# uci-rendering/psdr-cuda

Measured on AMD Instinct MI355X. Metric: Mpath-samples/s renderC+renderD, cbox 512x512 spp=64; grad rel-L2 vs ref, higher is better.
Workload: dtype f32

## Files before the change

psdr-cuda_amd/csrc/psdr_device.h:

```cpp
#pragma once
#include "psdr_math.h"
#include "../../include/psdr_hip.h"

namespace psdr {

struct __attribute__((aligned(16))) BvhNode {
    float lo0[3], hi0[3];
    float lo1[3], hi1[3];
    int32_t c0, c1;
    int32_t pad[2];
};
static_assert(sizeof(BvhNode) == 64, "BvhNode must be 64 bytes");

struct __attribute__((aligned(16))) Bvh4Node {
    float org[3];
    uint32_t exps;
    uint32_t qlo[3], qhi[3];
    int32_t child[4];
    uint32_t pad[2];
};
static_assert(sizeof(Bvh4Node) == 64, "Bvh4Node must be 64 bytes");
constexpr int32_t kNoChild = 0x7ffffffe;

constexpr int kBvhStack = 40;
// ... 980 lines not shown
    const float iw = 1.f / v[3];
    const Vec3f d = normalize(Vec3f{v[0] * iw, v[1] * iw, v[2] * iw});
    const float *c = sc.d.cam + PSDR_CAM_TO_WORLD;
    constexpr auto tm = &psdr_tangents::d_cam_to_world;
    auto tw = [&](int r, int col) { if constexpr (is_ad<R>()) return ldf<R>(c, tv, tm, r * 4 + col); else return R(uniform_word(c, r * 4 + col)); };
    RayT<R> ray;
    const R w = tw(3, 3);
    ray.o = Vec3<R>(tw(0, 3) / w, tw(1, 3) / w, tw(2, 3) / w);
    ray.d = Vec3<R>(tw(0, 0) * d.x + tw(0, 1) * d.y + tw(0, 2) * d.z, tw(1, 0) * d.x + tw(1, 1) * d.y + tw(1, 2) * d.z,
                    tw(2, 0) * d.x + tw(2, 1) * d.y + tw(2, 2) * d.z);
    return ray;
}
PSDR_HD bool sample_direct(const SceneView &sc, const Vec3f &p, int &pixel, float &qx, float &qy, float &sensor_val) {
    const float *m = sc.d.cam + PSDR_CAM_WORLD_TO_SAMPLE;
    float v[4];
#pragma unroll
    for (int r = 0; r < 4; ++r) v[r] = m[r * 4] * p.x + m[r * 4 + 1] * p.y + m[r * 4 + 2] * p.z + m[r * 4 + 3];
    qx = v[0] / v[3]; qy = v[1] / v[3];
    const int W = sc.d.width, H = sc.d.height;
    const int ix = (int) floorf(qx * (float) W), iy = (int) floorf(qy * (float) H);
    const bool ok = ix >= 0 && ix < W && iy >= 0 && iy < H;
    pixel = ok ? iy * W + ix : -1;
    const float *c = sc.d.cam;
    Vec3f dir{p.x - c[PSDR_CAM_POS], p.y - c[PSDR_CAM_POS + 1], p.z - c[PSDR_CAM_POS + 2]};
    const float d2 = dot(dir, dir);
    dir = dir / sqrtf(fmaxf(d2, 0.f));
    const float ict = 1.f / (c[PSDR_CAM_DIR] * dir.x + c[PSDR_CAM_DIR + 1] * dir.y + c[PSDR_CAM_DIR + 2] * dir.z);
    sensor_val = (1.f / d2) * (ict * ict * ict) * c[PSDR_CAM_INV_AREA];
    return ok;
}

#ifndef PSDR_EMITTER_PRETEST
#define PSDR_EMITTER_PRETEST 1
#endif
#ifndef PSDR_SKIP_UNLIT
#define PSDR_SKIP_UNLIT 1
#endif
#ifndef PSDR_OCC_ROWS
#define PSDR_OCC_ROWS 1
#endif
template <class R> PSDR_HD R mis_weight(const R &p1, const R &p2) { const R a = sqr(p1), b = sqr(p2); return a / (a + b); }

struct LiParams {
    int integrator, bsdf_samples, light_samples, max_depth, hide_emitters, field;
};

template <class R> PSDR_HD void copy_its(Its<R> &d, const Its<R> &a) {
    d.valid = a.valid; d.tri = a.tri; d.mesh = a.mesh; d.hu = a.hu; d.hv = a.hv;
    d.wi.x = a.wi.x; d.wi.y = a.wi.y; d.wi.z = a.wi.z; d.p.x = a.p.x; d.p.y = a.p.y; d.p.z = a.p.z; d.n.x = a.n.x; d.n.y = a.n.y; d.n.z = a.n.z;
    d.t = a.t; d.J = a.J; d.uvx = a.uvx; d.uvy = a.uvy;
    d.sh.s.x = a.sh.s.x; d.sh.s.y = a.sh.s.y; d.sh.s.z = a.sh.s.z; d.sh.t.x = a.sh.t.x; d.sh.t.y = a.sh.t.y; d.sh.t.z = a.sh.t.z;
    d.sh.n.x = a.sh.n.x; d.sh.n.y = a.sh.n.y; d.sh.n.z = a.sh.n.z;
}
template <class NI, class G> PSDR_HD NI its_cast(const Its<G> &a) {
    if constexpr (std::is_same<NI, Its<G>>::value) { if constexpr (is_ad<G>()) { NI r; copy_its(r, a); return r; } else return a; }
    else {
        Its<float> r;
        r.valid = a.valid; r.tri = a.tri; r.mesh = a.mesh; r.hu = a.hu; r.hv = a.hv;
        r.wi = val(a.wi); r.p = val(a.p); r.n = val(a.n); r.t = val(a.t); r.J = val(a.J); r.uvx = val(a.uvx); r.uvy = val(a.uvy);
        r.sh.s = val(a.sh.s); r.sh.t = val(a.sh.t); r.sh.n = val(a.sh.n);
        return r;
    }
}
template <class G, class M, class TVT, class NI = Its<G>>
PSDR_HD Vec3<M> direct_step(const SceneView &sc, const TVT &tv, TraversalStack &st, Rng &rng, const Its<G> &its, bool active, int nB,
                            int nL, uint32_t &nrays, NI *next_its, Vec3<M> *next_f, bool *next_valid, int *light_tri = nullptr, bool emitter_only = false) {
    constexpr bool ad = is_ad<M>();
    constexpr HitForm form = is_ad<G>() ? kPathSpace : kDetached;
    Vec3<M> result = zero3<M>();
    int bsdf_id = active ? Tab<TVT::flags>::mesh_bsdf(sc, its.mesh) : 0;
    if (bsdf_id < 0) { active = false; bsdf_id = 0; }
    const Bsdf<G, M> bsdf(sc, tv, bsdf_id);
    auto bsdf_sample = [&](const float (&s)[3], int i) {
        Vec3f wo_s; M pdf_s;
        bool a1 = bsdf.sample(sc, tv, its, s, active, wo_s, pdf_s);
        const Vec3f dir1 = val(its.sh.s) * wo_s.x + val(its.sh.t) * wo_s.y + val(its.sh.n) * wo_s.z;
        if constexpr (!TVT::has_env && TVT::forest && PSDR_EMITTER_PRETEST && !is_ad<G>()) {
            if (emitter_only && sc.emit_rows != 0u && a1) a1 = closest_hit<false, 2, true>(sc, st, val(its.p), dir1, INFINITY, -1, -1, 0, sc.emit_rows).tri >= 0;
        }
        const RayT<G> ray1{its.p, lift<G>(dir1)};
        const Its<G> its1 = intersect<G>(sc, tv, st, ray1, a1, form, nrays, -1, -1, kPreBsdfRay);
        const bool a_hit = a1 && its1.valid;
        a1 = a_hit && emitter_of(sc, tv, its1) >= 0;
        Vec3<M> bsdf_val = zero3<M>(); M pdf0(0.f);
        if (a_hit) {
            if constexpr (ad) {
                const Vec3<G> wo = (its1.p - its.p) / its1.t;
                bsdf_val = bsdf.eval(sc, tv, its, its.sh.to_local(wo), true);
                const G Gv = abs_(dot(its1.n, -wo)) / sqr(its1.t);
                pdf0 = pdf_s * val(Gv);
                bsdf_val = bsdf_val * (to_m<M>(Gv * its1.J) / pdf0);
            } else {
                bsdf_val = bsdf.eval(sc, tv, its, lift<G>(wo_s), true);
                const G Gv = abs_(dot(its1.n, -ray1.d)) / sqr(its1.t);
                pdf0 = pdf_s * Gv;
                bsdf_val = bsdf_val / pdf_s;
            }
        }
        if (a1) {
            M w(1.f / (float) nB);
            if (nL > 0) w = w * mis_weight(pdf0, M(emitter_position_pdf(sc, tv, val(its.p), its1)));
            result = result + Le<M>(sc, tv, its1, true) * bsdf_val * w;
        }
        if (next_its && i == 0) { *next_its = its_cast<NI>(its1); *next_f = bsdf_val; *next_valid = a_hit; }
    };
    auto light_sample = [&](float s0, float s1, int i) {
        const PosSample<G> ps = sample_emitter_position<G>(sc, tv, val(its.p), s0, s1, is_ad<G>());
        Vec3<G> wo = ps.p - its.p;
// ... 106 lines not shown
    const float ix = rho.x.v != 0.f ? 1.f / rho.x.v : 0.f, iy = rho.y.v != 0.f ? 1.f / rho.y.v : 0.f, iz = rho.z.v != 0.f ? 1.f / rho.z.v : 0.f;
#pragma unroll
    for (int k = 0; k < K; ++k) { g[k][0] = rho.x.d[k] * ix; g[k][1] = rho.y.d[k] * iy; g[k][2] = rho.z.d[k] * iz; }
}
template <int K, class TVT>
PSDR_HD Vec3<Dual<K>> li_path_logd(const SceneView &sc, const TVT &tv, TraversalStack &st, const LiParams &lp, Rng &rng, const RayT<float> &ray, uint32_t &nrays) {
    const TangentView<0, TVT::flags> tv0{};
    Its<float> its = intersect<float>(sc, tv0, st, ray, true, kDetached, nrays, -1, -1, kPrePrimaryRay);
    bool active = its.valid;
    Vec3f result = lp.hide_emitters ? Vec3f(0.f) : Le<float>(sc, tv0, its, active);
    float rd[K][3], s[K][3];
#pragma unroll
    for (int k = 0; k < K; ++k) { rd[k][0] = rd[k][1] = rd[k][2] = 0.f; s[k][0] = s[k][1] = s[k][2] = 0.f; }
    Vec3f beta(1.f);
    for (int depth = 0; depth < lp.max_depth; ++depth) {
        Its<float> nits; Vec3f nf; bool nvalid = false;
        if (active) {
            float g[K][3];
            albedo_logd<K>(sc, tv, its, g);
#pragma unroll
            for (int k = 0; k < K; ++k) { s[k][0] += g[k][0]; s[k][1] += g[k][1]; s[k][2] += g[k][2]; }
        }
        const Vec3f c = direct_step<float, float>(sc, tv0, st, rng, its, active, 1, 1, nrays, &nits, &nf, &nvalid, nullptr, depth + 1 >= lp.max_depth);
        if (active) {
            const Vec3f bc = beta * c;
            result = result + bc;
#pragma unroll
            for (int k = 0; k < K; ++k) {
                rd[k][0] = fmaf(bc.x, s[k][0], rd[k][0]); rd[k][1] = fmaf(bc.y, s[k][1], rd[k][1]); rd[k][2] = fmaf(bc.z, s[k][2], rd[k][2]);
            }
            active = nvalid;
            if (active) {
                beta = beta * nf;
                its = nits;
                if (!(beta.x != 0.f || beta.y != 0.f || beta.z != 0.f)) active = false;
            }
        }
    }
    Vec3<Dual<K>> out;
    out.x.v = result.x; out.y.v = result.y; out.z.v = result.z;
#pragma unroll
    for (int k = 0; k < K; ++k) { out.x.d[k] = rd[k][0]; out.y.d[k] = rd[k][1]; out.z.d[k] = rd[k][2]; }
    return out;
}
template <int K, class TVT>
PSDR_HD Vec3<Dual<K>> camera_sample_logd(const SceneView &sc, const TVT &tv, TraversalStack &st, const LiParams &lp, const RngJump &jump, int pixel, uint64_t slot, uint32_t &nrays) {
    Rng rng; rng.init(slot, jump);
    const float j0 = rng.next(), j1 = rng.next();
    const int W = sc.d.width;
    const float sx = ((float) (pixel % W) + j0) / (float) W, sy = ((float) (pixel / W) + j1) / (float) sc.d.height;
    const TangentView<0, TVT::flags> tv0{};
    const RayT<float> ray = primary_ray<float>(sc, tv0, sx, sy);
    return zero_nonfinite(li_path_logd<K>(sc, tv, st, lp, rng, ray, nrays));
}


template <class M, class TVT>
PSDR_HD Vec3<M> wavefront_camera_vertex(const SceneView &sc, const TVT &tv, TraversalStack &st, const LiParams &lp, const RngJump &jump,
                                        int pixel, uint64_t slot, uint32_t &nrays, Its<float> &next, Vec3<M> &beta, Vec3f &origin, bool &alive, Rng *rng_after = nullptr) {
    Rng rng; rng.init(slot, jump);
    const float j0 = rng.next(), j1 = rng.next();
    const int W = sc.d.width;
    const float sx = ((float) (pixel % W) + j0) / (float) W, sy = ((float) (pixel / W) + j1) / (float) sc.d.height;
    const RayT<float> ray = primary_ray<float>(sc, tv, sx, sy);
    const Its<float> its = intersect<float>(sc, tv, st, ray, true, kDetached, nrays);
    alive = false;
    if (!its.valid) return zero3<M>();
    Vec3<M> result = lp.hide_emitters ? zero3<M>() : Le<M>(sc, tv, its, true);
    bool nvalid = false;
    result = result + direct_step<float, M>(sc, tv, st, rng, its, true, 1, 1, nrays, &next, &beta, &nvalid, nullptr, lp.max_depth <= 1);
    if (rng_after) *rng_after = rng;
    origin = its.p;
    if (nvalid) { const Vec3f b = val(beta); alive = b.x != 0.f || b.y != 0.f || b.z != 0.f; }
    return result;
}
template <class M, class TVT>
PSDR_HD Vec3<M> wavefront_primary_vertex(const SceneView &sc, const TVT &tv, TraversalStack &st, const LiParams &lp, const RngJump &jump,
                                         int pixel, uint64_t slot, uint32_t &nrays, Its<float> &next, Vec3f &dir, bool &alive, Rng *rng_after = nullptr, float *sxy = nullptr) {
    Rng rng; rng.init(slot, jump);
    const float j0 = rng.next(), j1 = rng.next();
    if (rng_after) *rng_after = rng;
    const int W = sc.d.width;
    const float sx = ((float) (pixel % W) + j0) / (float) W, sy = ((float) (pixel / W) + j1) / (float) sc.d.height;
    if (sxy) { sxy[0] = sx; sxy[1] = sy; }
    const RayT<float> ray = primary_ray<float>(sc, tv, sx, sy);
    const Its<float> its = intersect<float>(sc, tv, st, ray, true, kDetached, nrays);
    alive = its.valid;
    if (!its.valid) return zero3<M>();
    next = its;
    { const Vec3f d = its.p - ray.o; dir = d / norm(d); }
    return lp.hide_emitters ? zero3<M>() : Le<M>(sc, tv, its, true);
}
template <class G> PSDR_HD Its<float> detach_its(const Its<G> &a) {
    Its<float> r;
    r.valid = a.valid; r.tri = a.tri; r.mesh = a.mesh; r.hu = a.hu; r.hv = a.hv;
    r.wi = val(a.wi); r.p = val(a.p); r.n = val(a.n); r.t = val(a.t); r.J = val(a.J); r.uvx = val(a.uvx); r.uvy = val(a.uvy);
    r.sh.s = val(a.sh.s); r.sh.t = val(a.sh.t); r.sh.n = val(a.sh.n);
    return r;
}
template <class M, class TVT>
PSDR_HD Vec3<M> wavefront_bounce_vertex(const SceneView &sc, const TVT &tv, TraversalStack &st, const RngJump &jump_k, uint64_t slot,
                                        const Its<float> &its, uint32_t &nrays, Its<float> &next, Vec3<M> &f, bool &alive, int *light_tri = nullptr,
                                        Rng *rng_after = nullptr, bool last = false) {
    Rng rng; rng.init(slot, jump_k);
    bool nvalid = false;
    if (light_tri) *light_tri = -1;
// ... 257 lines not shown
```

psdr-cuda_amd/csrc/psdr_hip.hip:

```cpp
#define PSDR_WIDE_TREE 2
#include "psdr_host.h"
#include "psdr_bvh_build.h"

#include <cstdlib>
#include <cstring>
#include <rocprim/rocprim.hpp>

namespace {
__global__ __launch_bounds__(kBlock) void k_trace(LaunchCtx cx, int m, const float *__restrict__ ox, const float *__restrict__ oy,
                                                  const float *__restrict__ oz, const float *__restrict__ dx,
                                                  const float *__restrict__ dy, const float *__restrict__ dz,
                                                  const float *__restrict__ tmax, int32_t *__restrict__ out_shape,
                                                  int32_t *__restrict__ out_tri, float *__restrict__ out_u, float *__restrict__ out_v) {
    TraversalStack st; setup_lds(cx, st);
    const SceneView &sc = cx.sc;
    for (int i = blockIdx.x * kBlock + threadIdx.x; i < m; i += gridDim.x * kBlock) {
        const Hit h = closest_hit<false, -1>(sc, st, Vec3f{ox[i], oy[i], oz[i]}, Vec3f{dx[i], dy[i], dz[i]}, tmax[i]);
        out_tri[i] = h.tri;
        out_shape[i] = h.tri >= 0 ? (sc.d.tri_mesh[h.tri] & ~PSDR_TRI_FACE_NORMALS) : -1;
        out_u[i] = h.u; out_v[i] = h.v;
    }
}


// ... 784 lines not shown
    HIP_TRY(hipMemsetAsync(pb.count, 0, cnt_bytes, s));
    return 0;
}

const VariantOps *variant_of(const psdr_scene_s *h) {
    int fl = (h->desc.env_emitter >= 0 ? kSceneEnv : 0) | (h->has_rough ? kSceneRough : 0) | (h->n_blas > 0 ? kSceneForest : 0);
    if (tiny_tables_ok(h)) fl |= kSceneTiny;
    switch (fl) {
        case 0: return variant_ops_0();
        case 1: return variant_ops_1();
        case 2: return variant_ops_2();
        case 3: return variant_ops_3();
        case 4: return variant_ops_4();
        case 8: return variant_ops_8();
        case 10: return variant_ops_10();
        default: return variant_ops_6();
    }
}
}
using namespace psdr_host;

extern "C" {

const char *psdr_last_error(void) { return g_err.c_str(); }
const char *psdr_version(void) { return "psdr-hip 0.1 gfx950"; }
int psdr_abi_struct_sizes(int32_t out[4]) {
    out[0] = (int32_t) sizeof(psdr_scene_desc); out[1] = (int32_t) sizeof(psdr_render_opts);
    out[2] = (int32_t) sizeof(psdr_tangents); out[3] = (int32_t) sizeof(psdr_grads);
    return 0;
}

int psdr_scene_create(psdr_scene_t *out) {
    if (!out) return fail("psdr_scene_create: null output");
    psdr_scene_s *h = new psdr_scene_s();
    hipError_t e = hipMalloc(&h->d_counters, sizeof(unsigned long long) * kRayCounters * kRayCounterStride);
    if (e != hipSuccess) { delete h; return fail(std::string("hipMalloc: ") + hipGetErrorString(e)); }
    int dev = 0; hipDeviceProp_t prop;
    if (hipGetDevice(&dev) == hipSuccess && hipGetDeviceProperties(&prop, dev) == hipSuccess) {
        h->num_cus = prop.multiProcessorCount;
        h->lds_limit = (int) std::min<size_t>(prop.sharedMemPerBlock, 160 * 1024);
    }
    *out = h;
    return 0;
}

int psdr_scene_set_option(psdr_scene_t h, const char *name, double value) {
    if (!h || !name) return fail("psdr_scene_set_option: null argument");
    const std::string n(name);
    const int iv = (int) value;
    if (n == "bvh_refit") h->refit_enabled = iv != 0;
    else if (n == "forest_min_inline") { h->forest_min_inline = iv; h->have_bvh = false; }
    else if (n == "scratch_plain") g_scratch_plain = iv;
    else if (n == "own_pixels") h->opt.own_pixels = iv;
    else if (n == "emitter_pretest") h->opt.emitter_pretest = iv;
    else if (n == "occ_rows") { h->opt.occ_rows = iv; h->have_bvh = false; }
    else if (n == "aa_prims") { h->aa_enabled = iv != 0; h->have_bvh = false; }
    else if (n == "tiny_scene") h->tiny_enabled = iv != 0;
    else if (n == "two_level") h->two_level_enabled = iv != 0;
    else if (n == "wf_binned") h->wf_binned = iv != 0;
    else if (n == "wf_traced") h->traced_enabled = iv != 0;
    else if (n == "bvh_build") h->bvh_device_mode = iv;
    else if (n == "sort_edges") h->sort_edges = iv != 0;
    else if (n == "blocks_per_cu") h->opt.blocks_per_cu = iv;
    else if (n == "camera_blocks") h->opt.camera_blocks = iv;
    else if (n == "tiny_variants") h->opt.tiny_variants = iv;
    else if (n == "wide") h->opt.wide = iv;
    else if (n == "lds_budget") h->opt.lds_budget = iv;
    else if (n == "sink_rep") h->opt.sink_rep = std::max(1, std::min(16, iv));
    else if (n == "sink_private") h->opt.sink_private = iv;
    else if (n == "rev_split") h->opt.rev_split = iv;
    else if (n == "tangent_live") h->opt.tangent_live = iv;
    else if (n == "wf_geo") h->opt.wf_geo = iv;
    else if (n == "logd") h->opt.logd = iv;
    else if (n == "keep_records") h->opt.keep_records = iv;
    else if (n == "rev_sorted") h->opt.rev_sorted = iv;
    else if (n == "sedge_split") h->opt.sedge_split = iv;
    else if (n == "probe") h->opt.probe = iv;
    else if (n == "trace_wg2") h->opt.trace_wg2 = iv;
    else if (n == "chunk_log2") h->opt.chunk_log2 = std::max(0, std::min(30, iv));
    else if (n == "bvh_maxleaf") h->opt.bvh_maxleaf = std::max(1, std::min(8, iv));
    else if (n == "bvh_tcost") h->opt.bvh_tcost = (float) value;
    else return fail("psdr_scene_set_option: unknown option '" + n + "'");
    h->kept.valid = false;
    if (n == "tiny_scene" || n == "two_level" || n == "bvh_build" || n == "wide" || n == "bvh_maxleaf" || n == "bvh_tcost" || n == "tiny_variants") h->have_bvh = false;
    return 0;
}

int psdr_scene_destroy(psdr_scene_t h) {
    if (!h) return 0;
    if (h->d_nodes) (void) hipFree(h->d_nodes);
    if (h->d_btris) (void) hipFree(h->d_btris);
    if (h->d_counters) (void) hipFree(h->d_counters);
    if (h->d_refit_area) (void) hipFree(h->d_refit_area);
    if (h->d_sort) (void) hipFree(h->d_sort);
    if (h->d_ws) (void) hipFree(h->d_ws);
    if (h->d_live) (void) hipFree(h->d_live);
    if (h->d_logd_bad) (void) hipFree(h->d_logd_bad);
    if (h->d_hot_map) (void) hipFree(h->d_hot_map);
    if (h->d_hot_tris) (void) hipFree(h->d_hot_tris);
    if (h->d_occ) (void) hipFree(h->d_occ);
    if (h->d_top) (void) hipFree(h->d_top);
    if (h->d_inline_ids) (void) hipFree(h->d_inline_ids);
    if (h->d_lbvh) (void) hipFree(h->d_lbvh);
    if (h->d_nodes4) (void) hipFree(h->d_nodes4);
    if (h->d_topo4) (void) hipFree(h->d_topo4);
    if (h->d_rev) (void) hipFree(h->d_rev);
// ... 371 lines not shown
```

psdr-cuda_amd/csrc/psdr_host.h:

```cpp
#pragma once
#include "psdr_device.h"
#include "psdr_reverse.h"

#include <algorithm>
#include <type_traits>
#include <cmath>
#include <cstdio>
#include <cstdlib>
#include <cstring>
#include <string>
#include <vector>

using namespace psdr;

struct LaunchCtx {
    SceneView sc;
    LiParams lp;
    RngJump jump;
    int32_t off_stack;
    int32_t off_pathrec;
    int32_t off_sink;
};

static_assert(offsetof(LaunchCtx, sc) == 0, "closest_hit reads SceneView::tiny through the kernel-argument segment pointer: LaunchCtx (SceneView first) must be the first kernel argument");
// ... 51 lines not shown
template <class TVT> __device__ __forceinline__ void setup_lds(const LaunchCtx &cx, TraversalStack &st, const TVT &tv) {
    setup_lds(cx, st);
#if defined(__HIP_DEVICE_COMPILE__)
    if constexpr (Tab<TVT::flags>::lds_small && TVT::k > 0) {
        constexpr int K = TVT::k;
        static_assert(K <= 3, "plan_lds reserves three tangent texel pools");
        if (cx.sc.lt_tex >= 0) {
            float *l = reinterpret_cast<float *>(psdr_dyn_lds + cx.sc.lt_tex);
            const int nt = cx.sc.d.num_texels;
            for (int k = 0; k < K; ++k) {
                const float *g = tv.t[k].d_texels;
                for (int i = threadIdx.x; i < nt; i += kBlock) l[(k + 1) * nt + i] = g ? g[i] : 0.f;
            }
            __syncthreads();
        }
    }
#endif
}

constexpr int kSinkCacheWords = 6144;
struct SinkLayout {
    int tex_off, tex_n;
    int rad_off, rad_n;
    int cam_off;
    int env_off, env_n;
    int hot_off, hot_rows;
    const int32_t *hot_map, *hot_tris;
    int total;
    int rep, stride;
    int priv_off, priv_rows;
    int priv_tri[2], priv_slot[2], priv_emitter;
    int priv_regs;
    int pend_off, pend_rows;
};
constexpr int kPendWords = 10;
constexpr int kPrivRowWords = 13;
constexpr int kPrivWords = 2 * kPrivRowWords + 3;

struct psdr_scene_options {
    int blocks_per_cu = 0;
    int camera_blocks = 0;
    int tiny_variants = 1;
    int wide = -1;
    int lds_budget = 0;
    int sink_rep = 4;
    int sink_private = 1;
    int rev_split = -1;
    int tangent_live = 1;
    int wf_geo = 1;
    int own_pixels = 1;
    int emitter_pretest = 1;
    int occ_rows = 1;
    int logd = 1;
    int keep_records = 1;
    int rev_sorted = 1;
    int sedge_split = -1;
    int chunk_log2 = 0;
    int probe = 1;
    int trace_wg2 = -1;
    int bvh_maxleaf = 4;
    float bvh_tcost = 2.0f;
};

struct psdr_scene_s {
    psdr_scene_options opt;
    psdr_scene_desc desc{};
    bool have_tables = false;
    bool has_rough = true;
    int num_cus = 256;
    int lds_limit = 64 * 1024;

    BvhNode *d_nodes = nullptr;
    float4 *d_btris = nullptr;
    size_t cap_nodes = 0, cap_btris = 0;
    int32_t root = 0;
    bool have_bvh = false;
    int bvh_depth = 0, num_nodes = 0, num_btris = 0;
    Bvh4Node *d_nodes4 = nullptr;
    int32_t *d_topo4 = nullptr;
    size_t cap_nodes4 = 0;
    int num_nodes4 = 0, stack_need4 = 0;
    bool wide = false;
    int32_t *d_trace_ovf = nullptr;
    size_t trace_ovf_bytes = 0;
    bool traced_enabled = true;
    int32_t root4 = 0, blas_root4[kMaxBlas] = {};
    bool refit_enabled = true;
    int tree_tris = -1, refits_since_build = 0, num_builds = 0, num_refits = 0;
    std::vector<int> level_start;
    float bvh_pad = 0.f, built_area = 0.f;
    float *d_refit_area = nullptr;

    int bvh_device_mode = -1;
    bool lbvh = false;
    int lbvh_leaves = 0;
    void *d_lbvh = nullptr;
    size_t lbvh_bytes = 0;

    bool tiny_enabled = true, aa_enabled = true;
    int n_tiny = 0, aa_cnt = 0;
    float4 tiny[kTinyRows * 4] = {};
    int32_t tiny_meta[kTinyRows * 4] = {};
    bool two_level_enabled = true, refit_ok = true, wf_binned = true;
    int n_blas = 0, n_inline = 0;
    float4 blas_lo[kMaxBlas] = {}, blas_hi[kMaxBlas] = {};
    float4 *d_top = nullptr;
// ... 92 lines not shown
```

psdr-cuda_amd/csrc/psdr_kernels.h:

```cpp
#pragma once
#include "psdr_host.h"

namespace {
using namespace psdr_host;

__device__ __forceinline__ float wave_shfl_down(float v, int off) { return __shfl_down(v, off, 64); }

template <int CTRL, int ROW_MASK> __device__ __forceinline__ float dpp_add(float v) {
    return v + __int_as_float(__builtin_amdgcn_update_dpp(0, __float_as_int(v), CTRL, ROW_MASK, 0xf, true));
}
__device__ __forceinline__ float wave_total(float v) {
    v = dpp_add<0x111, 0xf>(v); v = dpp_add<0x112, 0xf>(v); v = dpp_add<0x114, 0xf>(v); v = dpp_add<0x118, 0xf>(v);
    v = dpp_add<0x142, 0xa>(v); v = dpp_add<0x143, 0xc>(v);
    return __int_as_float(__builtin_amdgcn_readlane(__float_as_int(v), 63));
}
#ifndef PSDR_DPP_ALWAYS
#define PSDR_DPP_ALWAYS 0
#endif
template <int N, bool DPP = (N <= 6 || PSDR_DPP_ALWAYS)> __device__ __forceinline__ bool wave_segmented_sum(int key, float (&v)[N]) {
    const int lane = threadIdx.x & 63;
    if (DPP && __ballot(key != __builtin_amdgcn_readfirstlane(key)) == 0ull) {
#pragma unroll
        for (int i = 0; i < N; ++i) v[i] = wave_total(v[i]);
        return lane == 0;
// ... 147 lines not shown
    const int i = blockIdx.x * kBlock + threadIdx.x;
    bool b = false;
    if (i < n) {
        bool moved = false;
#pragma unroll
        for (int k = 0; k < K; ++k) moved = moved || tv.t[k].d_texels[i] != 0.f;
        b = moved && !(fabsf(texels[i]) > 1e-20f);
    }
    if (__ballot(b) != 0ull && (threadIdx.x & 63) == 0) atomicOr(bad, 1);
}
__global__ void k_logd_gate(unsigned long long *counters, const int *bad) { if (threadIdx.x == 0 && blockIdx.x == 0) counters[kLogdGateWord] = *bad ? 0ull : 1ull; }
template <int K, int FL, bool NOTREE>
__global__ __launch_bounds__(kBlock, ((PSDR_LOGD_WAVES_K1 > 0 && K == 1 && NOTREE) ? PSDR_LOGD_WAVES_K1 : camera_waves<float, Dual<K>, PSDR_INTEGRATOR_PATH, FL, NOTREE>())) void k_camera_logd(LaunchCtx cx, TV<Dual<K>, FL> tv, int spp, int s_begin, SlotDiv nsp,
                                                   long long n, float inv_spp, float *__restrict__ img, float *__restrict__ dimg, long long plane, unsigned long long *counters, int own) {
    constexpr int NV = 3 * (1 + K);
    if (counters[kLogdGateWord] != 1ull) return;
    TraversalStack st; setup_lds(cx, st, tv);
    uint32_t nrays = 0;
    const long long nceil = (n + kBlock - 1) / kBlock * kBlock;
    for (long long j = (long long) blockIdx.x * kBlock + threadIdx.x; j < nceil; j += (long long) gridDim.x * kBlock) {
        const bool in = j < n;
        int pixel = 0x7fffffff, s_in = 0;
        if (in) slot_to_pixel(j, nsp, pixel, s_in);
        float v[NV];
#pragma unroll
        for (int i = 0; i < NV; ++i) v[i] = 0.f;
        if (in) {
            const uint64_t slot = (uint64_t) pixel * (uint64_t) spp + (uint64_t) (s_begin + s_in);
            const Vec3<Dual<K>> r = camera_sample_logd<K>(cx.sc, tv, st, cx.lp, cx.jump, pixel, slot, nrays);
            v[0] = r.x.v * inv_spp; v[1] = r.y.v * inv_spp; v[2] = r.z.v * inv_spp;
#pragma unroll
            for (int k = 0; k < K; ++k) { v[3 + 3 * k] = r.x.d[k] * inv_spp; v[4 + 3 * k] = r.y.d[k] * inv_spp; v[5 + 3 * k] = r.z.d[k] * inv_spp; }
        }
        const bool head = wave_segmented_sum<NV>(pixel, v);
        if (head && in) {
            float *p = img + (size_t) pixel * 3;
            if (own) {
                p[0] = v[0]; p[1] = v[1]; p[2] = v[2];
#pragma unroll
                for (int k = 0; k < K; ++k) { float *q = dimg + (size_t) k * plane + (size_t) pixel * 3; q[0] = v[3 + 3 * k]; q[1] = v[4 + 3 * k]; q[2] = v[5 + 3 * k]; }
            } else {
                if (v[0] != 0.f) atomicAdd(p, v[0]);
                if (v[1] != 0.f) atomicAdd(p + 1, v[1]);
                if (v[2] != 0.f) atomicAdd(p + 2, v[2]);
#pragma unroll
                for (int k = 0; k < K; ++k) {
                    float *q = dimg + (size_t) k * plane + (size_t) pixel * 3;
                    if (v[3 + 3 * k] != 0.f) atomicAdd(q, v[3 + 3 * k]);
                    if (v[4 + 3 * k] != 0.f) atomicAdd(q + 1, v[4 + 3 * k]);
                    if (v[5 + 3 * k] != 0.f) atomicAdd(q + 2, v[5 + 3 * k]);
                }
            }
        }
    }
    count_rays(counters, nrays);
}

constexpr int kWfGroups = 16, kWfClasses = 4, kWfGrab = 8;
constexpr int kWfStageInts = (kWfSub + 1) * kWfCountStride;
struct PathStream {
    int32_t *pixel; uint32_t *slot; int32_t *tri; float *hu, *hv; float *dir; float *beta;
    float *acc;
    long long cap;
    int32_t *count;
    long long sub_cap;
    int32_t binned;
    float4 *hit;
    float *prev_t;
};
constexpr int kWfClsShift = 29;
constexpr int32_t kWfTriMask = (1 << kWfClsShift) - 1;
struct TraceQueue {
    float4 *req;
    int32_t *count;
    long long sub_cap;
};
struct WfRec {
    float *disk; long long stride;
    int spp, s_begin, nsp; long long j0;
    int stage;
    __device__ __forceinline__ long long column(int pixel, uint32_t slot) const {
        return (long long) pixel * nsp + (long long) (slot - (uint32_t) pixel * (uint32_t) spp - (uint32_t) s_begin) - j0;
    }
};

template <class M>
__device__ __forceinline__ void stream_write(const PathStream &out, long long i, int pixel, uint32_t slot, const Its<float> &next, const Vec3f &dir, const Vec3<M> &beta,
                                             const Vec3<M> &acc, int cls = 0) {
    constexpr int K = ad_traits<M>::K;
    out.pixel[i] = pixel; out.slot[i] = slot; out.tri[i] = next.tri | (cls << kWfClsShift); out.hu[i] = next.hu; out.hv[i] = next.hv;
    out.dir[i] = dir.x; out.dir[out.cap + i] = dir.y; out.dir[2 * out.cap + i] = dir.z;
    out.beta[i] = val(beta.x); out.beta[out.cap + i] = val(beta.y); out.beta[2 * out.cap + i] = val(beta.z);
    out.acc[i] = val(acc.x); out.acc[out.cap + i] = val(acc.y); out.acc[2 * out.cap + i] = val(acc.z);
#pragma unroll
    for (int k = 0; k < K; ++k) {
        out.beta[(3 + 3 * k) * out.cap + i] = tangent(beta.x, k); out.beta[(4 + 3 * k) * out.cap + i] = tangent(beta.y, k);
        out.beta[(5 + 3 * k) * out.cap + i] = tangent(beta.z, k);
        out.acc[(3 + 3 * k) * out.cap + i] = tangent(acc.x, k); out.acc[(4 + 3 * k) * out.cap + i] = tangent(acc.y, k);
        out.acc[(5 + 3 * k) * out.cap + i] = tangent(acc.z, k);
    }
}

template <class M>
__device__ __forceinline__ void stream_push(const PathStream &out, bool alive, int pixel, uint32_t slot, const Its<float> &next,
                                            const Vec3f &dir, const Vec3<M> &beta, const Vec3<M> &acc) {
    const unsigned long long mask = __ballot(alive);
// ... 1207 lines not shown
int run_camera(psdr_scene_s *h, const psdr_render_opts *o, const TV<R, FL> &tv, float *img, float *dimg, hipStream_t s) {
    const long long WH = (long long) h->desc.width * h->desc.height;
    const int nsp = o->spp_end - o->spp_begin;
    if (o->spp <= 0 || nsp <= 0) return 0;
    LaunchCtx cx;
    if (int rc = make_ctx(h, o, 0, cx)) return rc;
    const long long n = WH * nsp;
    h->slots[0] += (uint64_t) n;
    const int own = (h->opt.own_pixels != 0 && nsp <= 64 && 64 % nsp == 0) ? 1 : 0;
    if constexpr ((FL & kSceneForest) != 0) {
        if (o->integrator == PSDR_INTEGRATOR_DIRECT && probe_direct(h, o, n)) {
            const TangentView<0, FL> tv0{};
            TV<R, FL | kScenePre> tvp;
            for (int k = 0; k < (ad_traits<R>::K > 0 ? ad_traits<R>::K : 1); ++k) tvp.t[k] = tv.t[k];
            tvp.live = tv.live;
            LaunchCtx cxp = cx;
            plan_lds(h, cxp, 1 << 30);
            cxp.sc.n_lnodes = cxp.sc.n_lbtris = cxp.sc.n_ltri = 0;
            const long long chunk = std::min<long long>(n, launch_chunk(h, 25));
            for (long long c0 = 0; c0 < n; c0 += chunk) {
                const long long nc = std::min(chunk, n - c0);
                ProbeBuffers pb;
                const int probe_per_cu = big_launch_per_cu(h, nc);
                if (int rc = probe_buffers(h, nc, 3, pb, s, probe_per_cu)) return rc;
                const TraceQueue tq{pb.req, pb.count, pb.sub_cap};
                const int blocks = (launch_blocks(h, nc, probe_per_cu) + kWfSub - 1) / kWfSub * kWfSub;
                hipLaunchKernelGGL(k_direct_probe<FL>, dim3(blocks), dim3(kBlock), lds_bytes(cx, h), s, cx, tv0, o->spp, o->spp_begin, SlotDiv(nsp), c0, nc, tq, pb.hit, pb.mask,
                                   make_rng_jump(o->rng_offset[0] + 2));
                HIP_TRY(hipGetLastError());
                if (int rc = launch_wf_trace(h, pb.req, pb.count, pb.sub_cap, pb.hit, s)) return rc;
                hipLaunchKernelGGL(HIP_KERNEL_NAME(k_camera<G, R, PSDR_INTEGRATOR_DIRECT, FL | kScenePre, false>), dim3(launch_blocks(h, nc, camera_blocks_per_cu(h, nc))), dim3(kBlock), cxp.off_stack, s,
                                   cxp, tvp, o->spp, o->spp_begin, SlotDiv(nsp), nc, 1.f / (float) o->spp, img, dimg, WH * 3, h->d_counters, c0, ProbeView{pb.hit, pb.mask}, own);
                HIP_TRY(hipGetLastError());
            }
            return 0;
        }
    }
    bool gated = false;
    if constexpr (logd_instance<G, R, PSDR_INTEGRATOR_PATH, FL>()) {
        constexpr int K = ad_traits<R>::K;
        bool texels_only = o->integrator == PSDR_INTEGRATOR_PATH && h->opt.logd != 0 && h->desc.num_texels > 0 && h->desc.texels != nullptr;
        for (int k = 0; k < K && texels_only; ++k) {
            const psdr_tangents &t = tv.t[k];
            texels_only = t.d_texels != nullptr && !t.d_tri_info && !t.d_emitter_rad && !t.d_cam_to_world && !t.d_sec_edge && !t.d_prim_edge && !t.d_env_f;
        }
        if (texels_only) {
            if (int rc = scratch_reserve(&h->d_logd_bad, &h->logd_bad_bytes, sizeof(int), s, "log-derivative gate")) return rc;
            int *bad = reinterpret_cast<int *>(h->d_logd_bad);
            HIP_TRY(hipMemsetAsync(bad, 0, sizeof(int), s));
            TangentView<K, 0> tvk;
            for (int k = 0; k < K; ++k) tvk.t[k] = tv.t[k];
            hipLaunchKernelGGL(k_logd_check<K>, dim3((unsigned) ((h->desc.num_texels + kBlock - 1) / kBlock)), dim3(kBlock), 0, s, h->desc.texels, tvk, h->desc.num_texels, h->d_counters, bad);
            hipLaunchKernelGGL(k_logd_gate, dim3(1), dim3(64), 0, s, h->d_counters, bad);
            hipLaunchKernelGGL(HIP_KERNEL_NAME(k_camera_logd<K, FL, ((FL & kSceneTiny) != 0)>), dim3(launch_blocks(h, n, camera_blocks_per_cu(h, n))), dim3(kBlock), lds_bytes(cx, h), s, cx, tv,
                               o->spp, o->spp_begin, SlotDiv(nsp), n, 1.f / (float) o->spp, img, dimg, WH * 3, h->d_counters, own);
            HIP_TRY(hipGetLastError());
            gated = true;
        }
    }
#define PSDR_LAUNCH_CAMERA_T(INTEG, NOTREE)                                                                                        \
    hipLaunchKernelGGL(HIP_KERNEL_NAME(k_camera<G, R, INTEG, FL, NOTREE>), dim3(launch_blocks(h, n, camera_blocks_per_cu(h, n))), dim3(kBlock), lds_bytes(cx, h), s, cx, tv, o->spp, \
                       o->spp_begin, nsp, n, 1.f / (float) o->spp, img, dimg, WH * 3, h->d_counters, 0ll, ProbeView{nullptr, nullptr}, own)
#define PSDR_LAUNCH_CAMERA(INTEG) PSDR_LAUNCH_CAMERA_T(INTEG, ((FL & kSceneTiny) != 0))
    switch (o->integrator) {
        case PSDR_INTEGRATOR_DIRECT: PSDR_LAUNCH_CAMERA(PSDR_INTEGRATOR_DIRECT); break;
        case PSDR_INTEGRATOR_PATH: PSDR_LAUNCH_CAMERA(PSDR_INTEGRATOR_PATH); break;
        case PSDR_INTEGRATOR_FIELD: PSDR_LAUNCH_CAMERA(PSDR_INTEGRATOR_FIELD); break;
        default: return fail("Unknown integrator");
    }
#undef PSDR_LAUNCH_CAMERA
#undef PSDR_LAUNCH_CAMERA_T
    HIP_TRY(hipGetLastError());
    if (gated) HIP_TRY(hipMemsetAsync(h->d_counters + kLogdGateWord, 0, sizeof(unsigned long long), s));
    return 0;
}


constexpr int kWfMaxDepth = 256;
struct WfRecArgs { float *disk; long long stride, c0, nc; };
template <class M, int FL>
int run_camera_wavefront(psdr_scene_s *h, const psdr_render_opts *o, const TV<M, FL> &tv, float *img, float *dimg, hipStream_t s, const WfRecArgs *rec = nullptr) {
    constexpr int K = ad_traits<M>::K;
    const long long WH = (long long) h->desc.width * h->desc.height;
    const int nsp = o->spp_end - o->spp_begin;
    if (o->spp <= 0 || nsp <= 0) return 0;
    const long long n_all = WH * nsp;
    const long long n = rec ? rec->nc : n_all;
    bool traced = false;
    if constexpr ((FL & kSceneForest) != 0) traced = traced_wavefront(h);
    const bool binned = !traced && (FL & kSceneForest) != 0 && h->n_blas > 0 && h->wf_binned;
    const int depth = o->max_depth;
    const size_t words = 8 + 6 * (1 + K) + (traced ? 8 : 0);
    const long long cap = rec ? n : std::min(n, fit_chunk(binned ? launch_chunk(h, 24) : launch_chunk(h, traced ? 26 : 25), 2 * words * 4 * 5 / 4 + (traced ? 80 : 0), 64u << 20, h->ws_bytes));
    const auto wf_per_cu = [&](long long slots) { return traced ? big_launch_per_cu(h, slots) : 16; };
    const long long max_blocks = ((long long) launch_blocks(h, cap, wf_per_cu(cap)) + kWfSub - 1) / kWfSub * kWfSub;
    const long long binned_sub_cap = (((cap + kBlock - 1) / kBlock + kWfSub) / kWfGroups + 2) * kBlock;
    const long long cap_alloc = ((binned ? binned_sub_cap * kWfSub : cap + max_blocks * kBlock) + 63) / 64 * 64;
    const size_t cnt_ints = (size_t) (kWfMaxDepth + 1) * kWfStageInts + (traced ? (size_t) (kWfMaxDepth + 1) * kWfSub * kWfCountStride : 0);
    const size_t cnt_bytes = cnt_ints * sizeof(int32_t);
    const size_t req_bytes = traced ? (size_t) 2 * cap_alloc * 2 * sizeof(float4) : 0;
    const size_t need = 2 * words * 4 * (size_t) cap_alloc + cnt_bytes + req_bytes;
    if (int rc = workspace_reserve(h, need, s)) return rc;
    int32_t *cnt = reinterpret_cast<int32_t *>(h->d_ws);
    int32_t *req_cnt = cnt + (size_t) (kWfMaxDepth + 1) * kWfStageInts;
    PathStream st[2];
    for (int i = 0; i < 2; ++i) {
        float *b = reinterpret_cast<float *>(reinterpret_cast<char *>(h->d_ws) + cnt_bytes) + (size_t) i * words * cap_alloc;
        const long long c = cap_alloc;
        st[i].cap = c;
        st[i].pixel = reinterpret_cast<int32_t *>(b); st[i].slot = reinterpret_cast<uint32_t *>(b + c); st[i].tri = reinterpret_cast<int32_t *>(b + 2 * c);
        st[i].hu = b + 3 * c; st[i].hv = b + 4 * c; st[i].dir = b + 5 * c; st[i].beta = b + 8 * c; st[i].acc = b + (8 + 3 * (1 + K)) * c;
        st[i].hit = traced ? reinterpret_cast<float4 *>(b + (8 + 6 * (1 + K)) * c) : nullptr;
        st[i].prev_t = nullptr;
        st[i].binned = binned ? 1 : 0;
    }
    TraceQueue tq{};
    tq.req = traced ? reinterpret_cast<float4 *>(reinterpret_cast<char *>(h->d_ws) + cnt_bytes + 2 * words * 4 * (size_t) cap_alloc) : nullptr;
// ... 558 lines not shown
```

Measured before the change: 19970.

## Add compact path-tracing camera kernels with reduced state for tiny scenes

Adds specialized camera kernels for the primal and log-derivative path integrators on tiny scenes without a tree or environment map. Between bounces they carry only a minimal next-hit record (tri, u, v) instead of a full intersection struct, and they can park the per-path derivative sums in LDS. The kernels set launch bounds and an SGPR cap to raise occupancy. This trades extra LDS traffic and a second code path to maintain for lower register pressure, and they are on by default via compact_path=3.

```diff
diff --git a/psdr-cuda_amd/csrc/psdr_device.h b/psdr-cuda_amd/csrc/psdr_device.h
--- a/psdr-cuda_amd/csrc/psdr_device.h
+++ b/psdr-cuda_amd/csrc/psdr_device.h
@@ -1056,8 +1056,10 @@
     d.sh.s.x = a.sh.s.x; d.sh.s.y = a.sh.s.y; d.sh.s.z = a.sh.s.z; d.sh.t.x = a.sh.t.x; d.sh.t.y = a.sh.t.y; d.sh.t.z = a.sh.t.z;
     d.sh.n.x = a.sh.n.x; d.sh.n.y = a.sh.n.y; d.sh.n.z = a.sh.n.z;
 }
+struct NextHit { int tri; float u, v; };
 template <class NI, class G> PSDR_HD NI its_cast(const Its<G> &a) {
-    if constexpr (std::is_same<NI, Its<G>>::value) { if constexpr (is_ad<G>()) { NI r; copy_its(r, a); return r; } else return a; }
+    if constexpr (std::is_same<NI, NextHit>::value) return NextHit{a.tri, a.hu, a.hv};
+    else if constexpr (std::is_same<NI, Its<G>>::value) { if constexpr (is_ad<G>()) { NI r; copy_its(r, a); return r; } else return a; }
     else {
         Its<float> r;
         r.valid = a.valid; r.tri = a.tri; r.mesh = a.mesh; r.hu = a.hu; r.hv = a.hv;
@@ -1270,6 +1272,90 @@
     const TangentView<0, TVT::flags> tv0{};
     const RayT<float> ray = primary_ray<float>(sc, tv0, sx, sy);
     return zero_nonfinite(li_path_logd<K>(sc, tv, st, lp, rng, ray, nrays));
+}
+
+template <int K> struct CompactResult { Vec3f v; float d[K > 0 ? K : 1][3]; };
+template <int K, bool PARK> struct PathSums {
+    static constexpr int kWords = 6 * K + 6;
+    float r[PARK ? 1 : kWords];
+    float *p;
+    PSDR_HD float &w(int i) { if constexpr (PARK) return p[i * kBlock]; else return r[i]; }
+    PSDR_HD float &s(int k, int c) { return w(3 * k + c); }
+    PSDR_HD float &rd(int k, int c) { return w(3 * (K + k) + c); }
+    PSDR_HD float &result(int c) { return w(6 * K + c); }
+    PSDR_HD float &beta(int c) { return w(6 * K + 3 + c); }
+};
+template <int K, bool PARK = false, class TVT>
+PSDR_HD CompactResult<K> li_path_compact(const SceneView &sc, const TVT &tv, TraversalStack &st, const LiParams &lp, Rng &rng, const RayT<float> &ray, uint32_t &nrays,
+                                         float *park = nullptr) {
+    static_assert(!TVT::forest && !TVT::has_env, "the compact path serves scenes without a tree or an environment map");
+    const TangentView<0, TVT::flags> tv0{};
+    Its<float> its = intersect<float>(sc, tv0, st, ray, true, kDetached, nrays, -1, -1, kPrePrimaryRay);
+    bool active = its.valid;
+    PathSums<K, PARK> ps;
+    ps.p = park;
+    {
+        const Vec3f le = lp.hide_emitters ? Vec3f(0.f) : Le<float>(sc, tv0, its, active);
+        ps.result(0) = le.x; ps.result(1) = le.y; ps.result(2) = le.z;
+    }
+#pragma unroll
+    for (int k = 0; k < K; ++k)
+#pragma unroll
+        for (int c = 0; c < 3; ++c) { ps.s(k, c) = 0.f; ps.rd(k, c) = 0.f; }
+    ps.beta(0) = 1.f; ps.beta(1) = 1.f; ps.beta(2) = 1.f;
+    NextHit nh;
+    Vec3f o;
+    for (int depth = 0; depth < lp.max_depth && active; ++depth) {
+        if (depth > 0) {
+            its.valid = false; its.tri = its.mesh = -1; its.J = 1.f; its.t = INFINITY;
+            fill_its_from_hit<float>(its, sc, tv0, Hit{nh.tri, nh.u, nh.v, 0.f}, RayT<float>{o, o}, kDetached);
+        }
+        if constexpr (K > 0) {
+            float g[K][3];
+            albedo_logd<K>(sc, tv, its, g);
+#pragma unroll
+            for (int k = 0; k < K; ++k) { ps.s(k, 0) += g[k][0]; ps.s(k, 1) += g[k][1]; ps.s(k, 2) += g[k][2]; }
+        }
+        Vec3f nf; bool nvalid = false;
+        const Vec3f c = direct_step<float, float>(sc, tv0, st, rng, its, true, 1, 1, nrays, &nh, &nf, &nvalid, nullptr, depth + 1 >= lp.max_depth);
+        const Vec3f bc(ps.beta(0) * c.x, ps.beta(1) * c.y, ps.beta(2) * c.z);
+        ps.result(0) = ps.result(0) + bc.x; ps.result(1) = ps.result(1) + bc.y; ps.result(2) = ps.result(2) + bc.z;
+#pragma unroll
+        for (int k = 0; k < K; ++k) {
+            ps.rd(k, 0) = fmaf(bc.x, ps.s(k, 0), ps.rd(k, 0)); ps.rd(k, 1) = fmaf(bc.y, ps.s(k, 1), ps.rd(k, 1)); ps.rd(k, 2) = fmaf(bc.z, ps.s(k, 2), ps.rd(k, 2));
+        }
+        active = nvalid;
+        if (active) {
+            const Vec3f b(ps.beta(0) * nf.x, ps.beta(1) * nf.y, ps.beta(2) * nf.z);
+            ps.beta(0) = b.x; ps.beta(1) = b.y; ps.beta(2) = b.z;
+            o = its.p;
+            if (!(b.x != 0.f || b.y != 0.f || b.z != 0.f)) active = false;
+        }
+    }
+    CompactResult<K> out;
+    out.v.x = ps.result(0); out.v.y = ps.result(1); out.v.z = ps.result(2);
+#pragma unroll
+    for (int k = 0; k < K; ++k) { out.d[k][0] = ps.rd(k, 0); out.d[k][1] = ps.rd(k, 1); out.d[k][2] = ps.rd(k, 2); }
+    return out;
+}
+template <int K, bool PARK = false, class TVT>
+PSDR_HD CompactResult<K> camera_sample_compact(const SceneView &sc, const TVT &tv, TraversalStack &st, const LiParams &lp, const RngJump &jump, int pixel, uint64_t slot, uint32_t &nrays,
+                                               float *park = nullptr) {
+    Rng rng; rng.init(slot, jump);
+    const float j0 = rng.next(), j1 = rng.next();
+    const int W = sc.d.width;
+    const float sx = ((float) (pixel % W) + j0) / (float) W, sy = ((float) (pixel / W) + j1) / (float) sc.d.height;
+    const TangentView<0, TVT::flags> tv0{};
+    const RayT<float> ray = primary_ray<float>(sc, tv0, sx, sy);
+    CompactResult<K> r = li_path_compact<K, PARK>(sc, tv, st, lp, rng, ray, nrays, park);
+    const bool fx = isfinite(r.v.x), fy = isfinite(r.v.y), fz = isfinite(r.v.z);
+    r.v.x = fx ? r.v.x : 0.f; r.v.y = fy ? r.v.y : 0.f; r.v.z = fz ? r.v.z : 0.f;
+#pragma unroll
+    for (int k = 0; k < K; ++k) {
+        r.d[k][0] = (fx && isfinite(r.d[k][0])) ? r.d[k][0] : 0.f; r.d[k][1] = (fy && isfinite(r.d[k][1])) ? r.d[k][1] : 0.f;
+        r.d[k][2] = (fz && isfinite(r.d[k][2])) ? r.d[k][2] : 0.f;
+    }
+    return r;
 }
 
 
diff --git a/psdr-cuda_amd/csrc/psdr_hip.hip b/psdr-cuda_amd/csrc/psdr_hip.hip
--- a/psdr-cuda_amd/csrc/psdr_hip.hip
+++ b/psdr-cuda_amd/csrc/psdr_hip.hip
@@ -860,6 +860,7 @@
     else if (n == "forest_min_inline") { h->forest_min_inline = iv; h->have_bvh = false; }
     else if (n == "scratch_plain") g_scratch_plain = iv;
     else if (n == "own_pixels") h->opt.own_pixels = iv;
+    else if (n == "compact_path") h->opt.compact_path = iv;
     else if (n == "emitter_pretest") h->opt.emitter_pretest = iv;
     else if (n == "occ_rows") { h->opt.occ_rows = iv; h->have_bvh = false; }
     else if (n == "aa_prims") { h->aa_enabled = iv != 0; h->have_bvh = false; }
diff --git a/psdr-cuda_amd/csrc/psdr_host.h b/psdr-cuda_amd/csrc/psdr_host.h
--- a/psdr-cuda_amd/csrc/psdr_host.h
+++ b/psdr-cuda_amd/csrc/psdr_host.h
@@ -127,6 +127,7 @@
     int emitter_pretest = 1;
     int occ_rows = 1;
     int logd = 1;
+    int compact_path = 3;
     int keep_records = 1;
     int rev_sorted = 1;
     int sedge_split = -1;
diff --git a/psdr-cuda_amd/csrc/psdr_kernels.h b/psdr-cuda_amd/csrc/psdr_kernels.h
--- a/psdr-cuda_amd/csrc/psdr_kernels.h
+++ b/psdr-cuda_amd/csrc/psdr_kernels.h
@@ -223,6 +223,84 @@
                 }
             }
         }
+    }
+    count_rays(counters, nrays);
+}
+
+#ifndef PSDR_WAVES_COMPACT
+#define PSDR_WAVES_COMPACT 7
+#endif
+#ifndef PSDR_SGPR_COMPACT
+#define PSDR_SGPR_COMPACT 96
+#endif
+#ifndef PSDR_PARK_SUMS
+#define PSDR_PARK_SUMS 1
+#endif
+template <int FL> constexpr bool compact_instance() { return FL == kSceneTiny; }
+template <int NV>
+__device__ __forceinline__ void splat_pixel(const float (&v)[NV], int pixel, bool own, float *__restrict__ img, float *__restrict__ dimg, long long plane) {
+    constexpr int K = NV / 3 - 1;
+    float *p = img + (size_t) pixel * 3;
+    if (own) {
+        p[0] = v[0]; p[1] = v[1]; p[2] = v[2];
+#pragma unroll
+        for (int k = 0; k < K; ++k) { float *q = dimg + (size_t) k * plane + (size_t) pixel * 3; q[0] = v[3 + 3 * k]; q[1] = v[4 + 3 * k]; q[2] = v[5 + 3 * k]; }
+    } else {
+#pragma unroll
+        for (int i = 0; i < NV; ++i) {
+            float *q = i < 3 ? p + i : dimg + (size_t) (i / 3 - 1) * plane + (size_t) pixel * 3 + i % 3;
+            if (v[i] != 0.f) atomicAdd(q, v[i]);
+        }
+    }
+}
+template <int FL>
+__global__ __launch_bounds__(kBlock, PSDR_WAVES_COMPACT) __attribute__((amdgpu_num_sgpr(PSDR_SGPR_COMPACT)))
+void k_camera_compact(LaunchCtx cx, TV<float, FL> tv, int spp, int s_begin, SlotDiv nsp, long long n, float inv_spp, float *__restrict__ img,
+                      unsigned long long *counters, int own) {
+    TraversalStack st; setup_lds(cx, st, tv);
+    uint32_t nrays = 0;
+    const uint32_t nceil = (uint32_t) ((n + kBlock - 1) / kBlock * kBlock);
+    for (uint32_t j = blockIdx.x * kBlock + threadIdx.x; j < nceil; j += gridDim.x * kBlock) {
+        const bool in = (long long) j < n;
+        int pixel = 0x7fffffff, s_in = 0;
+        if (in) slot_to_pixel(j, nsp, pixel, s_in);
+        float v[3] = {0.f, 0.f, 0.f};
+        if (in) {
+            const uint64_t slot = (uint64_t) pixel * (uint64_t) spp + (uint64_t) (s_begin + s_in);
+            const Vec3f r = camera_sample_compact<0>(cx.sc, tv, st, cx.lp, cx.jump, pixel, slot, nrays).v;
+            v[0] = r.x * inv_spp; v[1] = r.y * inv_spp; v[2] = r.z * inv_spp;
+        }
+        const bool head = wave_segmented_sum<3>(pixel, v);
+        if (head && in) splat_pixel<3>(v, pixel, own != 0, img, nullptr, 0);
+    }
+    count_rays(counters, nrays);
+}
+template <int K, int FL>
+__global__ __launch_bounds__(kBlock, PSDR_WAVES_COMPACT) __attribute__((amdgpu_num_sgpr(PSDR_SGPR_COMPACT)))
+void k_camera_logd_compact(LaunchCtx cx, TV<Dual<K>, FL> tv, int spp, int s_begin, SlotDiv nsp, long long n, float inv_spp, float *__restrict__ img,
+                           float *__restrict__ dimg, long long plane, unsigned long long *counters, int own) {
+    constexpr int NV = 3 * (1 + K);
+    if (counters[kLogdGateWord] != 1ull) return;
+    __shared__ float park[PSDR_PARK_SUMS ? 6 * K + 6 : 1][kBlock];
+    TraversalStack st; setup_lds(cx, st, tv);
+    uint32_t nrays = 0;
+    const uint32_t nceil = (uint32_t) ((n + kBlock - 1) / kBlock * kBlock);
+    for (uint32_t j = blockIdx.x * kBlock + threadIdx.x; j < nceil; j += gridDim.x * kBlock) {
+        const bool in = (long long) j < n;
+        int pixel = 0x7fffffff, s_in = 0;
+        if (in) slot_to_pixel(j, nsp, pixel, s_in);
+        float v[NV];
+#pragma unroll
+        for (int i = 0; i < NV; ++i) v[i] = 0.f;
+        if (in) {
+            const uint64_t slot = (uint64_t) pixel * (uint64_t) spp + (uint64_t) (s_begin + s_in);
+            const CompactResult<K> r = camera_sample_compact<K, PSDR_PARK_SUMS != 0>(cx.sc, tv, st, cx.lp, cx.jump, pixel, slot, nrays, &park[0][threadIdx.x]);
+            v[0] = r.v.x * inv_spp; v[1] = r.v.y * inv_spp; v[2] = r.v.z * inv_spp;
+#pragma unroll
+            for (int k = 0; k < K; ++k) { v[3 + 3 * k] = r.d[k][0] * inv_spp; v[4 + 3 * k] = r.d[k][1] * inv_spp; v[5 + 3 * k] = r.d[k][2] * inv_spp; }
+        }
+        const bool head = wave_segmented_sum<NV>(pixel, v);
+        if (head && in) splat_pixel<NV>(v, pixel, own != 0, img, dimg, plane);
     }
     count_rays(counters, nrays);
 }
@@ -1536,8 +1614,16 @@
             for (int k = 0; k < K; ++k) tvk.t[k] = tv.t[k];
             hipLaunchKernelGGL(k_logd_check<K>, dim3((unsigned) ((h->desc.num_texels + kBlock - 1) / kBlock)), dim3(kBlock), 0, s, h->desc.texels, tvk, h->desc.num_texels, h->d_counters, bad);
             hipLaunchKernelGGL(k_logd_gate, dim3(1), dim3(64), 0, s, h->d_counters, bad);
-            hipLaunchKernelGGL(HIP_KERNEL_NAME(k_camera_logd<K, FL, ((FL & kSceneTiny) != 0)>), dim3(launch_blocks(h, n, camera_blocks_per_cu(h, n))), dim3(kBlock), lds_bytes(cx, h), s, cx, tv,
-                               o->spp, o->spp_begin, SlotDiv(nsp), n, 1.f / (float) o->spp, img, dimg, WH * 3, h->d_counters, own);
+            bool compact = false;
+            if constexpr (K == 1 && compact_instance<FL>()) compact = (h->opt.compact_path & 2) != 0;
+            if (compact) {
+                if constexpr (K == 1 && compact_instance<FL>())
+                    hipLaunchKernelGGL(HIP_KERNEL_NAME(k_camera_logd_compact<K, FL>), dim3(launch_blocks(h, n, camera_blocks_per_cu(h, n))), dim3(kBlock), lds_bytes(cx, h), s, cx, tv,
+                                       o->spp, o->spp_begin, SlotDiv(nsp), n, 1.f / (float) o->spp, img, dimg, WH * 3, h->d_counters, own);
+            } else {
+                hipLaunchKernelGGL(HIP_KERNEL_NAME(k_camera_logd<K, FL, ((FL & kSceneTiny) != 0)>), dim3(launch_blocks(h, n, camera_blocks_per_cu(h, n))), dim3(kBlock), lds_bytes(cx, h), s, cx, tv,
+                                   o->spp, o->spp_begin, SlotDiv(nsp), n, 1.f / (float) o->spp, img, dimg, WH * 3, h->d_counters, own);
+            }
             HIP_TRY(hipGetLastError());
             gated = true;
         }
@@ -1546,7 +1632,13 @@
     hipLaunchKernelGGL(HIP_KERNEL_NAME(k_camera<G, R, INTEG, FL, NOTREE>), dim3(launch_blocks(h, n, camera_blocks_per_cu(h, n))), dim3(kBlock), lds_bytes(cx, h), s, cx, tv, o->spp, \
                        o->spp_begin, nsp, n, 1.f / (float) o->spp, img, dimg, WH * 3, h->d_counters, 0ll, ProbeView{nullptr, nullptr}, own)
 #define PSDR_LAUNCH_CAMERA(INTEG) PSDR_LAUNCH_CAMERA_T(INTEG, ((FL & kSceneTiny) != 0))
-    switch (o->integrator) {
+    bool compact = false;
+    if constexpr (!is_ad<G>() && !is_ad<R>() && compact_instance<FL>()) compact = o->integrator == PSDR_INTEGRATOR_PATH && (h->opt.compact_path & 1) != 0;
+    if (compact) {
+        if constexpr (!is_ad<G>() && !is_ad<R>() && compact_instance<FL>())
+            hipLaunchKernelGGL(HIP_KERNEL_NAME(k_camera_compact<FL>), dim3(launch_blocks(h, n, camera_blocks_per_cu(h, n))), dim3(kBlock), lds_bytes(cx, h), s, cx, tv, o->spp,
+                               o->spp_begin, SlotDiv(nsp), n, 1.f / (float) o->spp, img, h->d_counters, own);
+    } else switch (o->integrator) {
         case PSDR_INTEGRATOR_DIRECT: PSDR_LAUNCH_CAMERA(PSDR_INTEGRATOR_DIRECT); break;
         case PSDR_INTEGRATOR_PATH: PSDR_LAUNCH_CAMERA(PSDR_INTEGRATOR_PATH); break;
         case PSDR_INTEGRATOR_FIELD: PSDR_LAUNCH_CAMERA(PSDR_INTEGRATOR_FIELD); break;
```

Result: faster. 20380, median of 6 (+2.1%).
